# ChicyChen/LOCO-Edit

Hardware: AMD Instinct MI355X
Metric: edit-directions/sec (top-5 PMP-Jacobian SVD @256^2) + vT cos-sim vs ref (higher is better)
Workload: dtype bf16x3 (split-bf16 MFMA operands, fp32 accumulate + fp32 storage); 1 GPU; CelebA-HQ DDPM 256x256 top-5 local basis (l_eye-sized mask, L=2400), t=0.6T, 12 power iterations, one GPU; multi_gpu_form=single, probes_total=5, probes_per_gpu=5, kept=5, n_iter=12, mask_L=2400, weights=synthetic seed 0, streams=2

## Files before the change

include/loco_hip_diag.h:

```cpp
#ifndef LOCO_HIP_DIAG_H
#define LOCO_HIP_DIAG_H
#include "loco_hip.h"
#ifdef __cplusplus
extern "C" {
#endif

int  loco_bench_conv(loco_ctx* ctx, int32_t cin, int32_t cout, int32_t H, int32_t W, int32_t B, int32_t mode,
                     int32_t taps, int32_t tile, int32_t iters, float* ms_avg, void* stream);

typedef struct loco_conv_desc {
    int32_t struct_size;
    int32_t Cin, Cout, Hin, Win, B, taps;
    int32_t stride, upsample, zins, mode, cpg;
    int32_t transposed, accumulate, in_arena, pad;
    int32_t Cin2, cot_cpg;
    float   res_scale;
    int32_t st_cpg;
    const float *weight, *bias;
    const float *in, *bias2, *res;
    const float *prim, *sc, *sh, *mr, *gamma, *tst, *tc;
    const float *in2, *w2, *bias2nd;
    const float *cot_d, *cot_prim, *cot_sc, *cot_sh, *cot_mr, *cot_tc;
    float* out;
    const float *st_prim, *st_mr;
    float* st_out;
    int32_t pool2;
} loco_conv_desc;
int  loco_debug_conv(loco_ctx* ctx, const loco_conv_desc* desc, char* plan, int64_t cap, void* stream);

int64_t loco_debug_tensor(loco_ctx* ctx, const char* name, float* dst, int64_t cap, void* stream);

#ifdef __cplusplus
}
#endif
#endif
```

loco-edit_amd/csrc/engine.hip:

```cpp
#include <hip/hip_runtime.h>

#include <algorithm>
#include <array>
#include <cmath>
#include <cstdio>
#include <cstdlib>
#include <cstring>
#include <map>
#include <memory>
#include <thread>
#include <atomic>
#include <string>
#include <vector>

#include "../../include/loco_hip.h"
#ifdef LOCO_DIAG
#include "../../include/loco_hip_diag.h"
#endif
#include "kernels.h"
#include "program.h"
#ifdef LOCO_DIAG
#include "conv_plan_text.h"
#endif

// ... 49 lines not shown

struct Tens : TensPlan {
    float* keep = nullptr; size_t keep_floats = 0; int keep_ntile = 0;
};
struct NormP : NormPlan, NormW {
    bool ready = false;
};
struct Op : OpPlan, OpWeights {
    NormP n1, n2, nx;
    float *xK = nullptr, *xV = nullptr;
};

struct HostParam { std::vector<float> data; std::vector<int64_t> shape; bool loaded = false; };

}


struct loco_ctx {
    loco_unet_cfg cfg;
    std::string err;
    std::map<std::string, HostParam> params;
    bool finalized = false;

    std::shared_ptr<const Program> prog;
    std::shared_ptr<Weights> wts;
    std::vector<Tens> tens;
    std::vector<Op> ops;


    float *arenaP = nullptr, *arenaT = nullptr;
    float *statsP = nullptr, *statsT = nullptr;
    double* red = nullptr;
    bool fuse_cot = true;
    float *stpart = nullptr, *stpart2 = nullptr;
    size_t stpart_floats = 0;
    bool fuse_stats = true;
    bool fuse_xattn = true;
    bool deep1 = true;
    bool flash_attn = true;
    float* attn_delta = nullptr;
    float* partial = nullptr;
    size_t partial_floats = 0;
    const float* bench_out = nullptr; int64_t bench_out_count = 0;
#ifdef LOCO_DIAG
    std::string* plan_log = nullptr;
#endif
    float *tact = nullptr, *tproj = nullptr;
    float* eps_buf = nullptr;
    float* gx0 = nullptr;
    float* ge = nullptr;
    float* tmpA = nullptr;
    double *G = nullptr, *Q = nullptr, *W = nullptr, *gscratch = nullptr;
    float* alphas = nullptr;
    float* ctx_colbias = nullptr;
    bool has_ctx = false;
    float* cond_add = nullptr;
    float* ctx_norm = nullptr;
    bool has_cond = false;
    float* cond_in = nullptr;
    bool has_tcond = false;
    float2* sxcache = nullptr;
    int prec = 0;
    std::vector<float*> owned;
    size_t bytes = 0;

    bool primal_ok = false;
// ... 477 lines not shown
#endif
    if (rq && rq->kind != ST_NONE && rq->n) rq->n->ready = true;
    if (rq && rq->keep_ntile) *rq->keep_ntile = p.keep_ntile;
    const int HWo = a.Hout * a.Wout, Gn = c->cfg.gn_groups;
    const long SBs = c->prog->stats_per_sample;
    auto timed = [&](const char* name, double flops, const ConvArgs& y, auto&& launch) {
        loco_ctx::ProfRec r;
        if (c->prof_on) {
            r.name = name; r.flops = flops;
            r.cin = y.Cin; r.cout = y.Cout; r.h = y.Hout; r.b = y.B; r.ns = y.nsplit; r.mode = y.mode; r.taps = taps;
            r.e0 = c->next_event(); r.e1 = c->next_event();
            (void)hipEventRecord(r.e0, st);
        }
        launch();
        if (c->prof_on) { (void)hipEventRecord(r.e1, st); c->prof.push_back(r); }
    };
    for (int li = 0; li < p.nl; ++li) {
        const ConvLaunch& l = p.l[li];
        const ConvArgs& x = l.args;
        double flops = 2.0 * (x.Cin * taps + x.Cin2) * x.Cout * (double)x.Hout * x.Wout * x.B;
        if (x.zins) flops *= 0.25;
        if (x.poly == 2) flops *= 4.0;
        timed(c->prof_on ? conv_variant_name(x, taps, c->prec) : nullptr, flops, x, [&] {
            if (c->prec == 1) launch_conv_bf16x3(x, taps, st);
            else if (c->prec == 2) launch_conv_f16(x, taps, st);
            else launch_conv(x, taps, st);
        });
        if (x.nsplit > 1) {
            timed("conv_splitk_reduce", 0.0, x, [&] {
                if (l.stats != SR_SPLITK) { launch_conv_splitk_reduce(x, st); return; }
                const NormP& n = *rq->n;
                NS sp = nstats(c, c->statsP, n);
                NS so = nstats(c, rq->stats + (long)l.s0 * SBs, n);
                launch_conv_splitk_reduce_stats(x, rq->kind, Gn, eps_of(c, n), n.gamma, n.beta, so.mr, so.sc, so.sh, SBs, rq->ss_scale,
                                                rq->ss_shift, rq->prim, sp.sc, sp.sh, sp.mr, so.tst, so.tc, SBs, c->red, st);
            });
        }
        if (l.stats == SR_ALONE) stats_standalone(c, *rq, x.out, x.out_bs, x.B, HWo, l.s0, st);
        if (l.stats == SR_EPI) {
            const NormP& n = *rq->n;
            NS so = nstats(c, rq->stats + (long)l.s0 * SBs, n);
            if (rq->kind != ST_FWD) {
                NS sp = nstats(c, c->statsP, n);
                launch_gn_lin_fused_finalize(rq->kind, x.st_part, n.C, l.ntile, nullptr, 0, x.B, n.C, HWo, Gn, sp.mr, so.tst, so.tc,
                                             SBs, st);
            } else {
                launch_gn_fused_finalize(x.st_part, l.ntile, x.B, n.C, HWo, Gn, eps_of(c, n), n.gamma, n.beta, so.mr, so.sc, so.sh,
                                         SBs, rq->ss_scale, rq->ss_shift, st);
            }
        }
    }
    if (p.stats_all) stats_standalone(c, *rq, a.out, a.out_bs, a.B, HWo, 0, st);
    if (p.pool_after)
        launch_pool2x2_sum(a.pool_tmp, a.pool_tmp_bs, p.pool_out, p.pool_out_bs, p.pool_acc, a.B, a.Cout, a.Hout, a.Wout, st);
    return p.cot;
}

inline void setw(ConvArgs& a, const ConvP& p, bool dgrad) {
    a.w = dgrad ? p.wd : p.wf;
    a.wb = dgrad ? (const void*)p.wbd : (const void*)p.wbf;
    a.wh = dgrad ? (const void*)p.whd : (const void*)p.whf;
    const bool folded = p.wpb && p.poly_dgrad == dgrad;
    a.wpb = folded ? p.wpb : nullptr;
    a.wph = folded ? p.wph : nullptr;
    a.wqb = dgrad ? p.wqb : nullptr;
    a.wqh = dgrad ? p.wqh : nullptr;
}
// ... 904 lines not shown
    for (size_t i = 0; i < P.ops.size(); ++i) {
        const OpPlan& plan = P.ops[i];
        Op& v = c->ops[i];
        static_cast<OpPlan&>(v) = plan;
        static_cast<NormPlan&>(v.n1) = plan.n1; static_cast<NormPlan&>(v.n2) = plan.n2; static_cast<NormPlan&>(v.nx) = plan.nx;
        if (!plan.has_ctx_kv()) continue;
        const size_t kv = (size_t)P.tens[plan.in].C * P.ctx_Lp;
        if (dalloc(c, &v.xK, kv) || dalloc(c, &v.xV, kv)) return -1;
    }
    return 0;
}

int create_ctx(loco_ctx* c, const loco_unet_cfg* cfg, std::shared_ptr<const Program> prog) {
    c->cfg = *cfg;
    c->prog = std::move(prog);
    const size_t MB = (size_t)cfg->max_batch;
    {
        float *p0 = nullptr, *p1 = nullptr;
        if (dalloc(c, &p0, MB * c->prog->per_sample + 128) || dalloc(c, &p1, MB * c->prog->per_sample + 128)) return -1;
        c->arenaP = p0 + 64; c->arenaT = p1 + 64;
    }
    if (dalloc(c, &c->statsP, MB * c->prog->stats_per_sample) || dalloc(c, &c->statsT, MB * c->prog->stats_per_sample)) return -1;
    if (dalloc(c, &c->red, RED_BYTES) || dalloc(c, &c->red2, RED_BYTES)) return -1;
    if (alloc_state(c)) return -1;
    {
        c->stpart_floats = MB * (size_t)(c->prog->max_tensor / 64 + 1) * 2;
        if (dalloc(c, &c->stpart, c->stpart_floats) || dalloc(c, &c->stpart2, c->stpart_floats)) return -1;
        const char* e = getenv("LOCO_FUSE_STATS");
        c->fuse_stats = !(e && atoi(e) == 0);
        e = getenv("LOCO_FUSE_LIN");
        c->fuse_lin = !(e && atoi(e) == 0);
        e = getenv("LOCO_FUSE_COT");
        c->fuse_cot = !(e && atoi(e) == 0) && cfg->act == ACT_SILU;
        e = getenv("LOCO_DEEP1");
        c->deep1 = !(e && atoi(e) == 0);
        e = getenv("LOCO_FUSE_XATTN");
        c->fuse_xattn = !(e && atoi(e) == 0);
        const char* fa = getenv("LOCO_FLASH_ATTN");
        c->flash_attn = !(fa && atoi(fa) == 0);
        if (dalloc(c, &c->attn_delta, MB * (size_t)c->prog->attn_dmax)) return -1;
    }
    c->partial_floats = (size_t)64 << 20;
    if (dalloc(c, &c->partial, c->partial_floats)) return -1;
    if (dalloc(c, &c->xin_buf, MB * c->prog->n_in) || dalloc(c, &c->t_dev, 4)) return -1;
    if (dalloc(c, &c->eps_buf, MB * c->prog->n_out) || dalloc(c, &c->gx0, MB * c->prog->n_in) || dalloc(c, &c->ge, MB * c->prog->n_out))
        return -1;
    if (dalloc(c, &c->tmpA, (size_t)64 * c->prog->n_in)) return -1;
    if (dalloc(c, &c->G, 64 * 64) || dalloc(c, &c->Q, 64 * 64) || dalloc(c, &c->W, SOLVER_W_GATE + 1)) return -1;
    {
        size_t nblk = ((size_t)c->prog->n_in + 255) / 256;
        if (dalloc(c, &c->gscratch, nblk * 64 * 64 + 4096)) return -1;
    }
    if (dalloc(c, &c->alphas, 256) || dalloc(c, &c->cond_add, (size_t)cfg->ch * 4)) return -1;
    if (dalloc(c, &c->cond_in, (size_t)cfg->ch)) return -1;
    {
        float2* sx0 = nullptr;
        if (dalloc(c, &sx0, (size_t)c->prog->sx_total + 64)) return -1;
        c->sxcache = sx0 + 32;
    }
    {
        const char* e = getenv("LOCO_PRECISION");
        c->prec = (e && std::string(e) == "f32") ? 0 : (e && std::string(e) == "f16") ? 2 : 1;
    }
    if (dalloc(c, &c->mask2, (size_t)c->prog->n_out)) return -1;
    if (dalloc(c, &c->mask, (size_t)c->prog->n_out) || dalloc(c, &c->mask_idx, (size_t)c->prog->n_out) ||
        dalloc(c, &c->mask_L_dev, 4)) return -1;
// ... 695 lines not shown
    const int taps = d->taps, k = taps == 9 ? 3 : 1, B = d->B;
    if ((taps != 9 && taps != 1) || d->Cin < 1 || d->Cout < 1 || d->Hin < 1 || d->Win < 1 || B < 1 || (d->stride != 1 && d->stride != 2) ||
        d->mode < CM_NONE || d->mode > CM_GN_GELU || (d->upsample && d->zins) || (d->stride == 2 && (d->upsample || d->zins)) ||
        !d->weight || !d->in || !d->out) { c->err = "debug_conv: bad descriptor"; return -2; }
    if (d->stride == 2 && ((d->Hin | d->Win) & 1)) { c->err = "debug_conv: stride 2 needs an even map"; return -2; }
    const bool lin = d->mode == CM_TAN_SILU || d->mode == CM_COT_SILU;
    if (d->mode != CM_NONE && (!d->sc || !d->sh)) { c->err = "debug_conv: the prologue modes need sc / sh"; return -2; }
    if (lin && (!d->prim || !d->mr || !d->gamma || !d->tst || !d->tc || d->cpg < 1 || d->Cin % d->cpg)) {
        c->err = "debug_conv: modes 3 / 4 need prim, mr, gamma, tst, tc and cpg"; return -2;
    }
    if (d->Cin2 > 0 && (!d->in2 || !d->w2)) { c->err = "debug_conv: the second operator needs in2 and w2"; return -2; }
    if (d->Cin2 > 0 && (d->res || d->accumulate || taps != 9)) {
        c->err = "debug_conv: the second operator goes with a 3x3 conv without res / accumulate"; return -2;
    }
    if (d->cot_d && (!d->cot_prim || !d->cot_sc || !d->cot_sh || !d->cot_mr || !d->cot_tc || d->cot_cpg < 1 || d->Cout % d->cot_cpg)) {
        c->err = "debug_conv: the norm-cotangent term needs cot_prim, cot_sc, cot_sh, cot_mr, cot_tc and cot_cpg"; return -2;
    }
    if (d->pool2 && (taps != 9 || d->stride != 1 || d->upsample || d->zins || d->mode != CM_NONE || d->Cin2 > 0 || d->res || d->cot_d ||
                     ((d->Hin | d->Win) & 1))) { c->err = "debug_conv: pool2 goes with a raw 3x3 stride-1 conv of an even map"; return -2; }
    const int Hout = (d->stride == 2 || d->pool2) ? d->Hin / 2 : (d->upsample || d->zins) ? 2 * d->Hin : d->Hin;
    const int Wout = (d->stride == 2 || d->pool2) ? d->Win / 2 : (d->upsample || d->zins) ? 2 * d->Win : d->Win;
    {
        auto pow2 = [](int v) { return v >= 8 && (v & (v - 1)) == 0; };
        auto walks = [&](int h, int w) { return (pow2(h) && pow2(w)) || (w % 32 == 0 && h % 8 == 0 && ((long)h * w) % 256 == 0); };
        if (!walks(Hout, Wout) || (d->pool2 && !walks(d->Hin, d->Win))) {
            c->err = "debug_conv: output map outside the tile geometry of the conv kernels"; return -2;
        }
    }
    const long in_e = (long)d->Cin * d->Hin * d->Win, out_e = (long)d->Cout * Hout * Wout, in2_e = (long)d->Cin2 * Hout * Wout;
    if ((in_e | out_e | in2_e) & 3) { c->err = "debug_conv: planes must be whole 16-byte units"; return -2; }
    auto up64 = [](long v) { return (v + 63) & ~63L; };
    const long offT_in2 = d->in_arena ? up64(in_e * B) : 0, offT_cot = offT_in2 + up64(in2_e * B);
    const long needT = offT_cot + (d->cot_d ? out_e * B : 0);
    const long sx_cot = lin ? up64(in_e) : 0, need_sx = sx_cot + (d->cot_d ? out_e : 0);
    if (needT > (long)c->cfg.max_batch * c->prog->per_sample || (lin && in_e > (long)c->cfg.max_batch * c->prog->per_sample) ||
        need_sx > c->prog->sx_total) { c->err = "debug_conv: shape exceeds the arenas"; return -2; }
    const int G = lin ? d->Cin / d->cpg : 0;
    const long tbs = up64(2L * G) + up64(2L * d->Cin);
    const bool st_req = d->st_prim != nullptr;
    if (st_req && (!d->st_mr || !d->st_out || d->st_cpg < 1 || d->Cout % d->st_cpg || d->cot_d || d->Cin2 > 0)) {
        c->err = "debug_conv: the statistics request needs st_prim, st_mr, st_out and st_cpg (no second operator, no cot_d)"; return -2;
    }
    const long keep_n = st_req ? up64((long)B * d->Cout * ((long)Hout * Wout / 64 + 1) * 2) : 0;
    const long small_n = (lin ? (long)B * tbs : 0) + (d->cot_d ? (long)B * up64(2L * d->Cout) : 0) + 64 + keep_n + (st_req ? up64(2L * d->Cout) : 0);
    const size_t owned0 = c->owned.size();
    const size_t bytes0 = c->bytes;
    auto release = [&]() {
        (void)hipStreamSynchronize(st);
        while (c->owned.size() > owned0) { (void)hipFree(c->owned.back()); c->owned.pop_back(); }
        c->bytes = bytes0;
    };
    auto host_param = [&](const float* p, std::vector<int64_t> shape) {
        HostParam h; h.shape = shape; h.loaded = true;
        size_t n = 1; for (int64_t s : shape) n *= (size_t)s;
        if (p) h.data.assign(p, p + n); else h.data.assign(n, 0.f);
        return h;
    };
    const int m_out = d->transposed ? d->Cin : d->Cout, m_in = d->transposed ? d->Cout : d->Cin;
    HostParam w = host_param(d->weight, {m_out, m_in, k, k}), wb0 = host_param(nullptr, {m_out});
    HostParam w2 = host_param(d->Cin2 > 0 ? d->w2 : nullptr, {d->Cout, d->Cin2 > 0 ? d->Cin2 : 1, 1, 1}), wb2 = host_param(nullptr, {d->Cout});
    ConvP cp, cp2;
    float *bias_d = nullptr, *bias2nd_d = nullptr, *small = nullptr;
    const int poly_kind = taps != 9 ? -1 : (d->upsample || d->pool2) ? POLY_UP : d->zins ? ((d->pad >= 0 ? d->pad : 2) == 1 ? POLY_ZINS_PAD1 : POLY_ZINS_PAD2) : -1;
    int rc = make_conv(c, {&w}, {&wb0}, &cp, -1, poly_kind, d->transposed != 0 && !d->pool2);
    float* pool_tmp = nullptr;
    if (!rc && d->pool2) rc = dalloc(c, &pool_tmp, (size_t)B * d->Cout * d->Hin * d->Win);
    if (!rc && d->Cin2 > 0) rc = make_conv(c, {&w2}, {&wb2}, &cp2);
// ... 31 lines not shown
        a.sx = c->sxcache;
    }
    ConvArgs n2; conv_defaults(n2);
    if (d->Cin2 > 0) {
        float* in2 = c->arenaT + offT_in2;
        if (he == hipSuccess) he = copy(in2, d->in2, in2_e * B);
        n2.in = in2; n2.in_bs = in2_e; n2.Cin = d->Cin2; n2.Hin = Hout; n2.Win = Wout;
        setw(n2, cp2, false); n2.bias = bias2nd_d; n2.pad = 0;
        n2.out = d->out; n2.out_bs = out_e; n2.Cout = d->Cout; n2.Hout = Hout; n2.Wout = Wout; n2.B = B;
        a.res = d->out; a.res_bs = out_e;
    }
    if (d->cot_d) {
        float* cd = c->arenaT + offT_cot;
        float* ctc = small + (lin ? (long)B * tbs : 0);
        const long cbs = up64(2L * d->Cout);
        if (he == hipSuccess) he = copy(cd, d->cot_d, out_e * B);
        for (int b = 0; b < B; ++b)
            hipLaunchKernelGGL(diag_scale_tc, dim3((unsigned)((d->Cout + 255) / 256)), dim3(256), 0, st, d->cot_tc + (long)b * 2 * d->Cout,
                               d->cot_mr, d->Cout, d->cot_cpg, (long)d->Cout, 1, ctc + b * cbs);
        launch_gn_cache(d->cot_prim, d->Cout, Hout * Wout, d->cot_cpg, d->cot_sc, d->cot_sh, d->cot_mr, c->sxcache + sx_cot, st, ACT_SILU);
        a.cot_d = cd; a.cot_d_bs = out_e; a.cot_sx = c->sxcache + sx_cot; a.cot_tc = ctc; a.cot_tc_bs = cbs;
    }
    if (he != hipSuccess) { c->err = std::string("debug_conv: ") + hipGetErrorString(he); release(); return -1; }
    std::string text;
    const int act0 = c->cfg.act;
    if (d->mode == CM_GN_GELU) c->cfg.act = ACT_GELU;
    c->plan_log = &text;
    StatReq srq;
    int kept_ntile = 0;
    float* const keep_buf = small + (small_n - keep_n - (st_req ? up64(2L * d->Cout) : 0));
    if (st_req) {
        srq.kind = ST_TAN; srq.prim = d->st_prim; srq.keep = keep_buf; srq.keep_floats = (size_t)keep_n; srq.keep_ntile = &kept_ntile;
    }
    const bool rode = run_conv(c, a, taps, st, st_req ? &srq : nullptr, d->Cin2 > 0 ? &n2 : nullptr);
    c->plan_log = nullptr;
    c->cfg.act = act0;
    if (st_req) {
        const int G2 = d->Cout / d->st_cpg;
        float* const zero = keep_buf + keep_n;
        (void)hipMemsetAsync(zero, 0, (size_t)up64(2L * d->Cout) * sizeof(float), st);
        (void)hipMemsetAsync(d->st_out, 0xff, (size_t)B * G2 * 2 * sizeof(float), st);
        if (kept_ntile > 0)
            launch_gn_lin_fused_finalize(ST_TAN, keep_buf, d->Cout, kept_ntile, nullptr, 0, B, d->Cout, Hout * Wout, G2, d->st_mr, d->st_out,
                                         nullptr, 2L * G2, st);
        launch_gn_tstats(d->out, out_e, d->st_prim, 0, B, d->Cout, Hout * Wout, G2, zero, zero + d->Cout, d->st_mr, 0, 0, 0,
                         d->st_out + (long)B * G2 * 2, nullptr, 2L * G2, c->red, st, ACT_SILU);
    }
    he = hipGetLastError();
    release();
    if (he == hipSuccess) he = hipGetLastError();
    if (he != hipSuccess) { c->err = std::string("debug_conv: ") + hipGetErrorString(he); return -1; }
    if (plan && cap > 0) {
        if ((int64_t)text.size() + 1 > cap) { c->err = "debug_conv: plan buffer too small"; return -4; }
        std::memcpy(plan, text.c_str(), text.size() + 1);
    }
    if (d->cot_d && !rode) { c->err = "debug_conv: norm-cotangent term declined"; return 1; }
    return 0;
}

#endif

int loco_set_streams(loco_ctx* c, int32_t n) {
    if (!c || (n != 1 && n != 2)) return -2;
    c->n_streams = n;
    return 0;
}

int loco_set_chip_share(loco_ctx* c, int32_t n) {
    if (!c || n < 1 || n > 8) return -2;
// ... 84 lines not shown
```

loco-edit_amd/csrc/misc.hip:

```cpp
#include "kernels.h"

namespace loco {

typedef float f32x4_t __attribute__((ext_vector_type(4)));

__device__ __forceinline__ double wave_sum(double v) {
#pragma unroll
    for (int o = 32; o > 0; o >>= 1) v += __shfl_down(v, o, 64);
    return v;
}
__device__ __forceinline__ float wave_sumf(float v) {
#pragma unroll
    for (int o = 32; o > 0; o >>= 1) v += __shfl_down(v, o, 64);
    return v;
}
__device__ __forceinline__ float wave_maxf(float v) {
#pragma unroll
    for (int o = 32; o > 0; o >>= 1) v = fmaxf(v, __shfl_down(v, o, 64));
    return v;
}
__device__ __forceinline__ double block_sum(double v, double* sm) {
    v = wave_sum(v);
    __syncthreads();
    if ((threadIdx.x & 63) == 0) sm[threadIdx.x >> 6] = v;
    __syncthreads();
    double r = 0.0;
    for (int i = 0; i < (int)(blockDim.x >> 6); ++i) r += sm[i];
    return r;
}

__global__ __launch_bounds__(256) void gn_partial_kernel(const float* x, long bs, long len, double* scratch) {
    __shared__ double sm[4];
    const int s = blockIdx.x, nsplit = gridDim.x, g = blockIdx.y, b = blockIdx.z, G = gridDim.y;
    const float* p = x + (long)b * bs + (long)g * len;
    long per = ((len / 4 + nsplit - 1) / nsplit) * 4;
    long beg = (long)s * per, end = beg + per < len ? beg + per : len;
    if (beg > end) beg = end;
    const long n4 = (end - beg) / 4;
    const float4* p4 = reinterpret_cast<const float4*>(p + beg);
    double sum = 0.0;
    for (long i = threadIdx.x; i < n4; i += 256) {
        float4 v = p4[i];
        sum += (double)((v.x + v.y) + (v.z + v.w));
    }
    for (long i = beg + n4 * 4 + threadIdx.x; i < end; i += 256) sum += (double)p[i];
    double tot = block_sum(sum, sm);
    const double cnt = (double)(end - beg);
    const float mean = cnt > 0 ? (float)(tot / cnt) : 0.f;
    double m2 = 0.0;
    for (long i = threadIdx.x; i < n4; i += 256) {
        float4 v = p4[i];
        float a0 = v.x - mean, a1 = v.y - mean, a2 = v.z - mean, a3 = v.w - mean;
        m2 += (double)((a0 * a0 + a1 * a1) + (a2 * a2 + a3 * a3));
    }
    for (long i = beg + n4 * 4 + threadIdx.x; i < end; i += 256) {
        float a0 = p[i] - mean;
        m2 += (double)(a0 * a0);
    }
    double M2 = block_sum(m2, sm);
    if (threadIdx.x == 0) {
        double* o = scratch + (((long)b * G + g) * nsplit + s) * 3;
// ... 286 lines not shown
        float* o = tst + (long)b * tbs + 2 * g;
        o[0] = m1;
        o[1] = m2;
    }
    if (tc) {
        const float f = kind == ST_TAN ? 1.0f : rstd;
        for (int k = threadIdx.x; k < cpg; k += 256) {
            float* t = tc + (long)b * tbs + 2 * ((long)g * cpg + k);
            t[0] = f * m1;
            t[1] = f * m2;
        }
    }
}
void launch_gn_lin_fused_finalize(int kind, const float* partA, int C1, int ntA, const float* partB, int ntB, int B, int C, int HW,
                                  int G, const float* mr, float* tst, float* tc, long tst_bs, hipStream_t st) {
    hipLaunchKernelGGL(gn_lin_fused_finalize_kernel, dim3(G, B), dim3(256), 0, st, kind, partA, C1, ntA, partB, ntB, C, G,
                       1.0 / ((double)(C / G) * HW), mr, tst, tc, tst_bs);
}
void launch_gn_fused_finalize_cat(const float* partA, int C1, int ntA, const float* partB, int ntB, int B, int C, int HW, int G,
                                  float eps, const float* gamma, const float* beta, float* mr, float* sc, float* sh,
                                  long stats_bs, hipStream_t st) {
    hipLaunchKernelGGL(gn_fused_finalize_cat_kernel, dim3(G, B), dim3(64), 0, st, partA, C1, ntA, partB, ntB, C, G, HW, eps,
                       gamma, beta, mr, sc, sh, stats_bs);
}

void launch_gn_fused_finalize(const float* part, int ntile, int B, int C, int HW, int G, float eps, const float* gamma,
                              const float* beta, float* mr, float* sc, float* sh, long stats_bs, const float* ss_scale,
                              const float* ss_shift, hipStream_t st) {
    const double inv_n = 1.0 / ((double)(C / G) * HW);
    hipLaunchKernelGGL(gn_fused_finalize_kernel, dim3(G, B), dim3(64), 0, st, part, ntile, C, G, inv_n, eps, gamma, beta, mr,
                       sc, sh, stats_bs, ss_scale, ss_shift);
}

template <int KIND>
__global__ __launch_bounds__(1024) void splitk_reduce_stats_kernel(ConvArgs a, int G, float eps, const float* gamma,
                                                                  const float* beta, float* mr, float* sc, float* sh, long sbs,
                                                                  const float* ss_scale, const float* ss_shift,
                                                                  const float* prim, const float* sc_p, const float* sh_p,
                                                                  const float* mr_p, float* tst, float* tc, long tbs,
                                                                  double* scratch) {
    __shared__ double sm[16];
    const int s = blockIdx.x, nsl = gridDim.x, g = blockIdx.y, b = blockIdx.z;
    const int HW = a.Hout * a.Wout, cpg = a.Cout / G;
    const long step = (long)blockDim.x * 4;
    const long len = (long)cpg * HW, per_b = (long)a.Cout * HW, total = per_b * a.B;
    const long base = (long)g * len;
    long per = ((len / 4 + nsl - 1) / nsl) * 4;
    long beg = (long)s * per, end = beg + per < len ? beg + per : len;
    if (beg > end) beg = end;
    float mean_p = 0.f, rstd_p = 1.f;
    if (KIND != ST_FWD) { mean_p = mr_p[2 * g]; rstd_p = mr_p[2 * g + 1]; }
    double t1 = 0.0, t2 = 0.0;
    for (long i = beg + threadIdx.x * 4; i < end; i += step) {
        const long e = base + i;
        const int c = (int)(e / HW);
        f32x4_t v = {0.f, 0.f, 0.f, 0.f};
        const float* pp = a.partial + (long)b * per_b + e;
        int k = 0;
        for (; k + 4 <= a.nsplit; k += 4) {
            const f32x4_t p0 = *reinterpret_cast<const f32x4_t*>(pp + (long)k * total);
            const f32x4_t p1 = *reinterpret_cast<const f32x4_t*>(pp + (long)(k + 1) * total);
            const f32x4_t p2 = *reinterpret_cast<const f32x4_t*>(pp + (long)(k + 2) * total);
            const f32x4_t p3 = *reinterpret_cast<const f32x4_t*>(pp + (long)(k + 3) * total);
            v += (p0 + p1) + (p2 + p3);
        }
        for (; k < a.nsplit; ++k) v += *reinterpret_cast<const f32x4_t*>(pp + (long)k * total);
        float add = 0.f;
        if (a.bias) add += a.bias[c];
        if (a.bias2) add += a.bias2[(long)b * a.bias2_bs + c];
        v += add;
        if (a.res) v += a.res_scale * *reinterpret_cast<const f32x4_t*>(a.res + (long)b * a.res_bs + e);
        float* o = a.out + (long)b * a.out_bs + e;
        if (a.accumulate) v += *reinterpret_cast<const f32x4_t*>(o);
        *reinterpret_cast<f32x4_t*>(o) = v;
        float a1, a2;
        if (KIND == ST_FWD) {
            a1 = (v[0] + v[1]) + (v[2] + v[3]);
            a2 = 0.f;
        } else {
            const f32x4_t xv = *reinterpret_cast<const f32x4_t*>(prim + e);
            const float scc = sc_p[c], shc = sh_p[c];
            a1 = 0.f; a2 = 0.f;
#pragma unroll
            for (int j = 0; j < 4; ++j) {
                const float xh = (xv[j] - mean_p) * rstd_p;
                float z = v[j];
                if (KIND == ST_COT) z *= (scc / rstd_p) * act_der(fmaf(scc, xv[j], shc), a.act);
                a1 += z;
                a2 += xh * z;
            }
        }
        t1 += (double)a1;
        t2 += (double)a2;
    }
    t1 = block_sum(t1, sm);
    if (KIND == ST_FWD) {
        const double n = (double)(end - beg);
        const float mu = n > 0 ? (float)(t1 / n) : 0.f;
        double m2 = 0.0;
        for (long i = beg + threadIdx.x * 4; i < end; i += step) {
            const f32x4_t v = *reinterpret_cast<const f32x4_t*>(a.out + (long)b * a.out_bs + base + i);
            const float d0 = v[0] - mu, d1 = v[1] - mu, d2 = v[2] - mu, d3 = v[3] - mu;
            m2 += (double)((d0 * d0 + d1 * d1) + (d2 * d2 + d3 * d3));
        }
        const double dm = (n > 0 ? t1 / n : 0.0) - (double)mu;
        t2 = block_sum(m2, sm) - n * dm * dm;
    } else {
        t2 = block_sum(t2, sm);
    }
    if (nsl > 1) {
        if (threadIdx.x == 0) {
            if (KIND == ST_FWD) {
                double* o = scratch + (((long)b * G + g) * nsl + s) * 3;
                const double n = (double)(end - beg), mu = n > 0 ? t1 / n : 0.0;
                o[0] = n; o[1] = mu; o[2] = t2;
            } else {
                double* o = scratch + (((long)b * G + g) * nsl + s) * 2;
                o[0] = t1; o[1] = t2;
            }
        }
        return;
    }
    const double inv_n = 1.0 / (double)len;
    if (KIND == ST_FWD) {
        const double mean = t1 * inv_n;
        double var = t2 * inv_n;
        if (var < 0.0) var = 0.0;
        const float meanf = (float)mean, rstd = (float)(1.0 / sqrt(var + (double)eps));
        if (threadIdx.x == 0) {
            mr[(long)b * sbs + g * 2] = meanf;
            mr[(long)b * sbs + g * 2 + 1] = rstd;
        }
        if (threadIdx.x < cpg) {
            const int c = g * cpg + threadIdx.x;
            const float gm = gamma[c];
            float aa = gm * rstd, oo = beta[c] - meanf * rstd * gm;
            if (ss_scale) {
                const float f = 1.0f + ss_scale[c];
                aa *= f;
                oo = oo * f + ss_shift[c];
            }
            sc[(long)b * sbs + c] = aa;
            sh[(long)b * sbs + c] = oo;
        }
    } else {
        const float m1 = (float)(t1 * inv_n), m2 = (float)(t2 * inv_n);
        if (threadIdx.x == 0) {
            tst[(long)b * tbs + 2 * g] = m1;
            tst[(long)b * tbs + 2 * g + 1] = m2;
        }
        if (tc && threadIdx.x < cpg) {
            const float f = KIND == ST_TAN ? 1.0f : rstd_p;
            float* t = tc + (long)b * tbs + 2 * ((long)g * cpg + threadIdx.x);
            t[0] = f * m1;
            t[1] = f * m2;
        }
    }
}

void launch_conv_splitk_reduce_stats(const ConvArgs& a, int kind, int G, float eps, const float* gamma, const float* beta,
                                     float* mr, float* sc, float* sh, long stats_bs, const float* ss_scale,
                                     const float* ss_shift, const float* prim, const float* sc_prim, const float* sh_prim,
                                     const float* mr_prim, float* tst, float* tc, long tst_bs, double* scratch,
                                     hipStream_t st) {
    const int HW = a.Hout * a.Wout, cpg = a.Cout / G;
    const long len = (long)cpg * HW;
    const int ns = gn_nsplit(len, a.B * G);
    dim3 grid(ns, G, a.B);
    long pieces = (len / ns + 3) / 4;
    int nthr = (int)((pieces + 63) / 64) * 64;
    if (nthr < 64) nthr = 64;
    if (nthr > 1024) nthr = 1024;
    if (nthr < cpg) nthr = ((cpg + 63) / 64) * 64;
#define RS(K) hipLaunchKernelGGL(splitk_reduce_stats_kernel<K>, grid, dim3(nthr), 0, st, a, G, eps, gamma, beta, mr, sc, sh, \
                                 stats_bs, ss_scale, ss_shift, prim, sc_prim, sh_prim, mr_prim, tst, tc, tst_bs, scratch)
    if (kind == ST_FWD) RS(ST_FWD); else if (kind == ST_TAN) RS(ST_TAN); else RS(ST_COT);
#undef RS
    if (ns == 1) return;
    if (kind == ST_FWD) {
        hipLaunchKernelGGL(gn_finalize_kernel, dim3((G + 63) / 64, a.B), dim3(64), 0, st, scratch, ns, G, a.Cout, eps, gamma,
                           beta, mr, sc, sh, stats_bs, ss_scale, ss_shift);
    } else {
        const long BG = (long)a.B * G;
        hipLaunchKernelGGL(gn_tstats_finalize, dim3((unsigned)((BG + 255) / 256)), dim3(256), 0, st, scratch, ns, BG, G,
                           1.0 / (double)len, tst, tc, tst_bs, cpg, mr_prim, 0L, kind == ST_TAN ? 0 : 1);
    }
}

template <int KIND>
__global__ __launch_bounds__(256) void gn_apply_kernel(const float* d, long d_bs, const float* x, long x_bs,
                                                       const float* base, long base_bs, float* out, long out_bs,
                                                       int accumulate, int C, int HW, int cpg, const float* sc,
                                                       const float* sh, const float* mr, long pbs_c, long pbs_g,
                                                       const float* tst, long tbs, int act, float base_scale) {
    const int b = blockIdx.y;
    const long per = (long)C * HW;
    for (long i = ((long)blockIdx.x * 256 + threadIdx.x) * 4; i < per; i += (long)gridDim.x * 1024) {
        int c = (int)(i / HW);
        int g = c / cpg;
        float scc = sc[(long)b * pbs_c + c], shc = sh[(long)b * pbs_c + c];
        float4 xv = *reinterpret_cast<const float4*>(x + (long)b * x_bs + i);
        float xx[4] = {xv.x, xv.y, xv.z, xv.w};
        float r[4];
        if (KIND == 0) {
#pragma unroll
            for (int j = 0; j < 4; ++j) r[j] = fmaf(scc, xx[j], shc);
        } else if (KIND == 4) {
#pragma unroll
            for (int j = 0; j < 4; ++j) r[j] = act_fwd(fmaf(scc, xx[j], shc), act);
// ... 439 lines not shown
```

loco-edit_amd/hip.py:

```python
from __future__ import annotations

import ctypes as C
import os
from typing import Dict, Optional

import numpy as np
import torch

from .config import UNetConfig

_LIB_PATH = os.environ.get("LOCO_HIP_LIB") or os.path.join(os.path.dirname(os.path.abspath(__file__)), "libloco_hip.so")
_lib = None

DIAG_SYMBOLS = ["loco_bench_conv", "loco_debug_conv", "loco_debug_tensor"]

SYMBOLS = [
    "loco_version", "loco_device_count", "loco_create", "loco_fork", "loco_destroy", "loco_last_error",
    "loco_load_param", "loco_params_missing", "loco_unet_forward", "loco_ddim_step", "loco_sched_step",
    "loco_pmp_primal", "loco_pmp_set_second_mask", "loco_pmp_jvp", "loco_pmp_vjp", "loco_orthonormalize", "loco_qr_rows",
    "loco_convergence", "loco_convergence_rows", "loco_null_project", "loco_edit_axpy", "loco_mask_gather", "loco_mask_count",
    "loco_unet_flops", "loco_workspace_bytes", "loco_clock_stamp", "loco_set_side_stream", "loco_timer_start", "loco_timer_stop",
    "loco_profile_enable", "loco_profile_report", "loco_set_precision", "loco_get_precision", "loco_set_streams", "loco_set_chip_share",
    "loco_set_cond", "loco_set_context", "loco_lincomb", "loco_masked_axpby", "loco_latent_sample",
    "loco_text_create", "loco_text_load_param", "loco_text_params_missing", "loco_text_encode", "loco_text_last_error",
    "loco_text_destroy", "loco_t5_create", "loco_text_encode_masked",
    "loco_diffedit_mask", "loco_cfg_masked_step", "loco_set_time_cond", "loco_lcm_step",
    "loco_sam_create", "loco_sam_load_param", "loco_sam_params_missing", "loco_sam_encode", "loco_sam_profile",
    "loco_sam_profile_read", "loco_sam_last_error", "loco_sam_destroy",
    "loco_samdec_create", "loco_samdec_load_param", "loco_samdec_params_missing", "loco_samdec_set_image", "loco_samdec_predict",
    "loco_samdec_score", "loco_samdec_binarize", "loco_samdec_last_error", "loco_samdec_destroy",
    "loco_clipvis_create", "loco_clipvis_load_param", "loco_clipvis_params_missing", "loco_clipvis_preprocess",
    "loco_clipvis_encode", "loco_clipvis_last_error", "loco_clipvis_destroy",
    "loco_quality_create", "loco_quality_load_param", "loco_quality_params_missing", "loco_quality_lpips", "loco_quality_ssim",
    "loco_quality_masked_mse", "loco_quality_last_error", "loco_quality_destroy",
]

DIFFEDIT_RULES = {"reference": 0, "intended": 1}


class LocoCfg(C.Structure):
    _fields_ = [
        ("struct_size", C.c_int32), ("resolution", C.c_int32), ("in_channels", C.c_int32), ("out_ch", C.c_int32), ("ch", C.c_int32),
        ("num_levels", C.c_int32), ("ch_mult", C.c_int32 * 8), ("num_res_blocks", C.c_int32),
        ("num_attn_res", C.c_int32), ("attn_resolutions", C.c_int32 * 8), ("gn_groups", C.c_int32),
        ("gn_eps", C.c_float), ("max_batch", C.c_int32),
        ("arch", C.c_int32), ("num_head_channels", C.c_int32), ("learn_sigma", C.c_int32),
        ("context_dim", C.c_int32), ("context_len", C.c_int32),
        ("scale_shift_norm", C.c_int32), ("resblock_updown", C.c_int32), ("num_heads", C.c_int32),
        ("transformer_depth", C.c_int32),
        ("act", C.c_int32), ("res_scale", C.c_float), ("added_kv", C.c_int32),
        ("time_cond_proj_dim", C.c_int32),
    ]


class LocoConvDesc(C.Structure):
    _PTRS = ("weight", "bias", "in", "bias2", "res", "prim", "sc", "sh", "mr", "gamma", "tst", "tc", "in2", "w2", "bias2nd",
             "cot_d", "cot_prim", "cot_sc", "cot_sh", "cot_mr", "cot_tc", "out", "st_prim", "st_mr", "st_out")
    _HOST = ("weight", "bias", "w2", "bias2nd")
    _fields_ = ([("struct_size", C.c_int32)] +
                [(k, C.c_int32) for k in ("Cin", "Cout", "Hin", "Win", "B", "taps", "stride", "upsample", "zins", "mode", "cpg",
                                          "transposed", "accumulate", "in_arena", "pad", "Cin2", "cot_cpg")] +
                [("res_scale", C.c_float), ("st_cpg", C.c_int32)] + [(k, C.c_void_p) for k in _PTRS] + [("pool2", C.c_int32)])


class LocoTextCfg(C.Structure):
    _fields_ = [("vocab", C.c_int32), ("width", C.c_int32), ("layers", C.c_int32), ("heads", C.c_int32), ("ffn", C.c_int32),
                ("positions", C.c_int32), ("act", C.c_int32), ("ln_eps", C.c_float)]


class LocoT5Cfg(C.Structure):
    _fields_ = [("vocab", C.c_int32), ("d_model", C.c_int32), ("d_kv", C.c_int32), ("heads", C.c_int32), ("d_ff", C.c_int32),
                ("layers", C.c_int32), ("positions", C.c_int32), ("buckets", C.c_int32), ("max_distance", C.c_int32),
                ("act", C.c_int32), ("ln_eps", C.c_float)]


SAM_MAX_GLOBAL = 16


class LocoSamCfg(C.Structure):
    _fields_ = [("image_size", C.c_int32), ("patch_size", C.c_int32), ("width", C.c_int32), ("depth", C.c_int32),
                ("heads", C.c_int32), ("mlp_dim", C.c_int32), ("window_size", C.c_int32), ("num_global", C.c_int32),
                ("global_attn", C.c_int32 * SAM_MAX_GLOBAL), ("out_channels", C.c_int32), ("ln_eps", C.c_float)]


class LocoSamDecCfg(C.Structure):
    _fields_ = [("grid", C.c_int32), ("image_size", C.c_int32), ("hidden", C.c_int32), ("layers", C.c_int32), ("heads", C.c_int32),
                ("mlp_dim", C.c_int32), ("attention_downsample_rate", C.c_int32), ("num_multimask_outputs", C.c_int32),
                ("iou_head_depth", C.c_int32), ("iou_head_hidden_dim", C.c_int32), ("layer_norm_eps", C.c_float),
                ("hidden_act", C.c_int32), ("max_prompts", C.c_int32)]


class LocoClipVisCfg(C.Structure):
    _fields_ = [("image_size", C.c_int32), ("patch_size", C.c_int32), ("width", C.c_int32), ("layers", C.c_int32),
                ("heads", C.c_int32), ("mlp_dim", C.c_int32), ("projection_dim", C.c_int32), ("act", C.c_int32),
                ("ln_eps", C.c_float), ("image_mean", C.c_float * 3), ("image_std", C.c_float * 3)]
# ... 553 lines not shown
            side = BranchStreams._pick(1, self.device)
            if not side:
                self.set_streams(1)
                return 1
            self.set_side_stream(side[0])
        self.set_streams(n)
        return n

    def get_precision(self) -> str:
        m = self.lib.loco_get_precision(self._ctx)
        return {v: k for k, v in self.PRECISIONS.items()}[m]

    def _need_diag(self, sym):
        if not hasattr(self.lib, sym):
            raise RuntimeError(f"{sym} is a diagnostic of include/loco_hip_diag.h: build `make -C loco-edit_amd/csrc diag` "
                               "and set LOCO_HIP_LIB=<repo>/loco-edit_amd/libloco_hip_diag.so")

    def bench_conv(self, cin, cout, H, W, B, mode, taps=9, tile=-1, iters=20) -> float:
        self._need_diag("loco_bench_conv")
        ms = C.c_float()
        self._check(self.lib.loco_bench_conv(self._ctx, cin, cout, H, W, B, mode, taps, tile, iters, C.byref(ms),
                                             _stream()), "loco_bench_conv")
        return float(ms.value)

    def debug_conv(self, out: torch.Tensor, **desc):
        self._need_diag("loco_debug_conv")
        d = LocoConvDesc()
        d.struct_size = C.sizeof(LocoConvDesc)
        d.stride, d.in_arena, d.pad, d.res_scale = 1, 1, -1, 1.0
        keep = []
        _chk_dev(out)
        d.out = out.data_ptr()
        for k, v in desc.items():
            if k not in LocoConvDesc._PTRS:
                if not hasattr(d, k) or k == "struct_size":
                    raise TypeError(f"debug_conv: no descriptor field {k!r}")
                setattr(d, k, v)
            elif v is not None:
                if k in LocoConvDesc._HOST:
                    v = v.detach().to("cpu", torch.float32).contiguous()
                else:
                    _chk_dev(v)
                keep.append(v)
                setattr(d, k, v.data_ptr())
        buf = C.create_string_buffer(1 << 12)
        rc = self.lib.loco_debug_conv(self._ctx, C.byref(d), buf, len(buf), _stream())
        if rc not in (0, 1):
            self._check(rc, "loco_debug_conv")
        plan = []
        for line in buf.value.decode().splitlines():
            rec = dict(f.split("=", 1) for f in line.split(" "))
            plan.append({k: (v if k == "kernel" else int(v)) for k, v in rec.items()})
        return plan, rc == 0

    def profile_enable(self, on):
        self._check(self.lib.loco_profile_enable(self._ctx, int(on)), "loco_profile_enable")

    def profile_report(self):
        buf = C.create_string_buffer(1 << 18)
        self._check(self.lib.loco_profile_report(self._ctx, buf, len(buf)), "loco_profile_report")
        out = {}
        for line in buf.value.decode().splitlines():
            name, n, ms, fl = line.rsplit(" ", 3)
            out[name] = dict(launches=int(float(n)), ms=float(ms), flops=float(fl))
        return out

    def debug_tensor(self, name: str, numel: int) -> torch.Tensor:
# ... 333 lines not shown
```

Measured before the change: 20.35 edit-directions/s.

## Overhaul split-K reduce-stats kernel: cached cotangent records, slab-templated loads, register reuse

Reworks the split-K reduce plus group-norm statistics kernel. It templates the number of partial slabs so all loads are issued up front. The cotangent path reads precomputed scale/x-hat records from the sx cache instead of recomputing the activation derivative. Forward mode keeps the first few reduced vectors in registers for the variance pass, and the two block sums are merged into one. It also replaces 64-bit division with shifts or 32-bit division and adds diagnostic hooks for the norm-stats path, at the cost of more template instances and extra register pressure.

```diff
diff --git a/include/loco_hip_diag.h b/include/loco_hip_diag.h
--- a/include/loco_hip_diag.h
+++ b/include/loco_hip_diag.h
@@ -25,6 +25,9 @@
     const float *st_prim, *st_mr;
     float* st_out;
     int32_t pool2;
+    int32_t sn_kind, sn_records;
+    const float *sn_gamma, *sn_beta, *sn_prim, *sn_sc, *sn_sh, *sn_mr;
+    float* sn_out;
 } loco_conv_desc;
 int  loco_debug_conv(loco_ctx* ctx, const loco_conv_desc* desc, char* plan, int64_t cap, void* stream);
 
diff --git a/loco-edit_amd/csrc/engine.hip b/loco-edit_amd/csrc/engine.hip
--- a/loco-edit_amd/csrc/engine.hip
+++ b/loco-edit_amd/csrc/engine.hip
@@ -105,6 +105,7 @@
     float *statsP = nullptr, *statsT = nullptr;
     double* red = nullptr;
     bool fuse_cot = true;
+    bool splitk_cot_rec = true;
     float *stpart = nullptr, *stpart2 = nullptr;
     size_t stpart_floats = 0;
     bool fuse_stats = true;
@@ -648,7 +649,10 @@
                 const NormP& n = *rq->n;
                 NS sp = nstats(c, c->statsP, n);
                 NS so = nstats(c, rq->stats + (long)l.s0 * SBs, n);
-                launch_conv_splitk_reduce_stats(x, rq->kind, Gn, eps_of(c, n), n.gamma, n.beta, so.mr, so.sc, so.sh, SBs, rq->ss_scale,
+                ConvArgs y = x;
+                y.st_sx = (rq->kind == ST_COT && c->splitk_cot_rec && c->prec >= 1 && n.sx_off >= 0 && c->sxcache) ? c->sxcache + n.sx_off
+                                                                                                                     : nullptr;
+                launch_conv_splitk_reduce_stats(y, rq->kind, Gn, eps_of(c, n), n.gamma, n.beta, so.mr, so.sc, so.sh, SBs, rq->ss_scale,
                                                 rq->ss_shift, rq->prim, sp.sc, sp.sh, sp.mr, so.tst, so.tc, SBs, c->red, st);
             });
         }
@@ -1619,6 +1623,8 @@
         c->fuse_lin = !(e && atoi(e) == 0);
         e = getenv("LOCO_FUSE_COT");
         c->fuse_cot = !(e && atoi(e) == 0) && cfg->act == ACT_SILU;
+        e = getenv("LOCO_SPLITK_COT_REC");
+        c->splitk_cot_rec = !(e && atoi(e) == 0);
         e = getenv("LOCO_DEEP1");
         c->deep1 = !(e && atoi(e) == 0);
         e = getenv("LOCO_FUSE_XATTN");
@@ -2380,7 +2386,16 @@
     auto up64 = [](long v) { return (v + 63) & ~63L; };
     const long offT_in2 = d->in_arena ? up64(in_e * B) : 0, offT_cot = offT_in2 + up64(in2_e * B);
     const long needT = offT_cot + (d->cot_d ? out_e * B : 0);
-    const long sx_cot = lin ? up64(in_e) : 0, need_sx = sx_cot + (d->cot_d ? out_e : 0);
+    const bool sn_req = d->sn_kind != ST_NONE;
+    const int Gn = c->cfg.gn_groups;
+    if (sn_req && (d->sn_kind < ST_FWD || d->sn_kind > ST_COT || d->Cout % Gn || !d->sn_out || d->st_prim || d->cot_d || d->Cin2 > 0 ||
+                   d->pool2 || (d->sn_kind == ST_FWD ? (!d->sn_gamma || !d->sn_beta) : (!d->sn_prim || !d->sn_sc || !d->sn_sh || !d->sn_mr)))) {
+        c->err = "debug_conv: the norm statistics request needs sn_out, Cout a multiple of the groups, sn_gamma / sn_beta (forward) or "
+                 "sn_prim, sn_sc, sn_sh, sn_mr (tangent, cotangent); no second operator, cot_d, st_prim or pool2";
+        return -2;
+    }
+    const bool sn_rec = sn_req && d->sn_kind == ST_COT && d->sn_records;
+    const long sx_cot = lin ? up64(in_e) : 0, need_sx = sx_cot + ((d->cot_d || sn_rec) ? out_e : 0);
     if (needT > (long)c->cfg.max_batch * c->prog->per_sample || (lin && in_e > (long)c->cfg.max_batch * c->prog->per_sample) ||
         need_sx > c->prog->sx_total) { c->err = "debug_conv: shape exceeds the arenas"; return -2; }
     const int G = lin ? d->Cin / d->cpg : 0;
@@ -2478,9 +2493,33 @@
     if (st_req) {
         srq.kind = ST_TAN; srq.prim = d->st_prim; srq.keep = keep_buf; srq.keep_floats = (size_t)keep_n; srq.keep_ntile = &kept_ntile;
     }
-    const bool rode = run_conv(c, a, taps, st, st_req ? &srq : nullptr, d->Cin2 > 0 ? &n2 : nullptr);
+    NormP dn;
+    float* const statsP0 = c->statsP;
+    const long sn_slot = 4L * d->Cout + 4L * Gn, SBs = c->prog->stats_per_sample;
+    float *sn_primal = nullptr, *sn_stats = nullptr;
+    if (sn_req) {
+        const size_t stats_n = (size_t)((B - 1) * SBs + sn_slot);
+        if (dalloc(c, &sn_primal, (size_t)sn_slot) || dalloc(c, &sn_stats, stats_n)) { c->plan_log = nullptr; c->cfg.act = act0; release(); return -1; }
+        dn.C = d->Cout; dn.soff = 0;
+        dn.gamma = const_cast<float*>(d->sn_gamma); dn.beta = const_cast<float*>(d->sn_beta);
+        (void)hipMemsetAsync(sn_stats, 0xff, stats_n * sizeof(float), st);
+        if (d->sn_kind != ST_FWD) {
+            NS sp = nstats(c, sn_primal, dn);
+            (void)copy(sp.sc, d->sn_sc, d->Cout); (void)copy(sp.sh, d->sn_sh, d->Cout); (void)copy(sp.mr, d->sn_mr, 2L * Gn);
+            if (sn_rec) {
+                launch_gn_cache(d->sn_prim, d->Cout, Hout * Wout, d->Cout / Gn, d->sn_sc, d->sn_sh, d->sn_mr, c->sxcache + sx_cot, st, c->cfg.act);
+                dn.sx_off = sx_cot;
+            }
+        }
+        srq.kind = d->sn_kind; srq.n = &dn; srq.stats = sn_stats; srq.prim = d->sn_prim;
+        c->statsP = sn_primal;
+    }
+    const bool rode = run_conv(c, a, taps, st, (st_req || sn_req) ? &srq : nullptr, d->Cin2 > 0 ? &n2 : nullptr);
+    c->statsP = statsP0;
     c->plan_log = nullptr;
     c->cfg.act = act0;
+    if (sn_req)
+        for (int b = 0; b < B; ++b) (void)copy(d->sn_out + (long)b * sn_slot, sn_stats + (long)b * SBs, sn_slot);
     if (st_req) {
         const int G2 = d->Cout / d->st_cpg;
         float* const zero = keep_buf + keep_n;
diff --git a/loco-edit_amd/csrc/misc.hip b/loco-edit_amd/csrc/misc.hip
--- a/loco-edit_amd/csrc/misc.hip
+++ b/loco-edit_amd/csrc/misc.hip
@@ -27,6 +27,17 @@
     double r = 0.0;
     for (int i = 0; i < (int)(blockDim.x >> 6); ++i) r += sm[i];
     return r;
+}
+__device__ __forceinline__ void block_sum2(double& a, double& b, double* sm) {
+    a = wave_sum(a);
+    b = wave_sum(b);
+    __syncthreads();
+    if ((threadIdx.x & 63) == 0) { sm[threadIdx.x >> 6] = a; sm[16 + (threadIdx.x >> 6)] = b; }
+    __syncthreads();
+    double ra = 0.0, rb = 0.0;
+    for (int i = 0; i < (int)(blockDim.x >> 6); ++i) { ra += sm[i]; rb += sm[16 + i]; }
+    a = ra;
+    b = rb;
 }
 
 __global__ __launch_bounds__(256) void gn_partial_kernel(const float* x, long bs, long len, double* scratch) {
@@ -379,14 +390,45 @@
                        sc, sh, stats_bs, ss_scale, ss_shift);
 }
 
-template <int KIND>
+constexpr int SPLITK_KEEP = 4;
+template <int NSLAB>
+__device__ __forceinline__ void splitk_load(const float* pp, long total, int k0, int nsplit, f32x4_t (&p)[NSLAB]) {
+#pragma unroll
+    for (int j = 0; j < NSLAB; ++j) {
+        const int k = k0 + j < nsplit ? k0 + j : nsplit - 1;
+        p[j] = *reinterpret_cast<const f32x4_t*>(pp + (long)k * total);
+    }
+}
+template <int NSLAB>
+__device__ __forceinline__ f32x4_t splitk_add(f32x4_t v, const f32x4_t (&p)[NSLAB], int k0, int nsplit) {
+    static_assert(NSLAB % 4 == 0, "whole groups of four");
+#pragma unroll
+    for (int j = 0; j < NSLAB; j += 4) {
+        if (k0 + j + 4 <= nsplit) v += (p[j] + p[j + 1]) + (p[j + 2] + p[j + 3]);
+        else {
+#pragma unroll
+            for (int r = 0; r < 4; ++r)
+                if (k0 + j + r < nsplit) v += p[j + r];
+        }
+    }
+    return v;
+}
+static int splitk_chunk(int nsplit) { return nsplit <= 4 ? 4 : nsplit <= 8 ? 8 : nsplit <= 12 ? 12 : 16; }
+static int splitk_pow2_shift(long v) {
+    if (v <= 0 || (v & (v - 1))) return -1;
+    int s = 0;
+    while ((1L << s) < v) ++s;
+    return s;
+}
+
+template <int KIND, int NSLAB>
 __global__ __launch_bounds__(1024) void splitk_reduce_stats_kernel(ConvArgs a, int G, float eps, const float* gamma,
                                                                   const float* beta, float* mr, float* sc, float* sh, long sbs,
                                                                   const float* ss_scale, const float* ss_shift,
                                                                   const float* prim, const float* sc_p, const float* sh_p,
-                                                                  const float* mr_p, float* tst, float* tc, long tbs,
-                                                                  double* scratch) {
-    __shared__ double sm[16];
+                                                                  const float* mr_p, const float2* sx_p, int hw_shift, float* tst,
+                                                                  float* tc, long tbs, double* scratch) {
+    __shared__ double sm[32];
     const int s = blockIdx.x, nsl = gridDim.x, g = blockIdx.y, b = blockIdx.z;
     const int HW = a.Hout * a.Wout, cpg = a.Cout / G;
     const long step = (long)blockDim.x * 4;
@@ -395,65 +437,122 @@
     long per = ((len / 4 + nsl - 1) / nsl) * 4;
     long beg = (long)s * per, end = beg + per < len ? beg + per : len;
     if (beg > end) beg = end;
+    const bool rec = KIND == ST_COT && sx_p != nullptr;
+    const bool idx32 = per_b <= 0x7fffffffL;
     float mean_p = 0.f, rstd_p = 1.f;
     if (KIND != ST_FWD) { mean_p = mr_p[2 * g]; rstd_p = mr_p[2 * g + 1]; }
-    double t1 = 0.0, t2 = 0.0;
-    for (long i = beg + threadIdx.x * 4; i < end; i += step) {
+    auto piece = [&](long i, float& a1, float& a2) -> f32x4_t {
         const long e = base + i;
-        const int c = (int)(e / HW);
+        const float* pp = a.partial + (long)b * per_b + e;
+        f32x4_t p[NSLAB];
+        splitk_load<NSLAB>(pp, total, 0, a.nsplit, p);
+        const int c = hw_shift >= 0 ? (int)(e >> hw_shift) : idx32 ? (int)((unsigned)e / (unsigned)HW) : (int)(e / HW);
+        float* o = a.out + (long)b * a.out_bs + e;
+        const float add = *(a.bias ? a.bias + c : pp);
+        const float add2 = *(a.bias2 ? a.bias2 + (long)b * a.bias2_bs + c : pp);
+        const f32x4_t rv = *reinterpret_cast<const f32x4_t*>(a.res ? a.res + (long)b * a.res_bs + e : pp);
+        const f32x4_t ov = *reinterpret_cast<const f32x4_t*>(a.accumulate ? o : pp);
+        float scc = 0.f, shc = 0.f;
+        f32x4_t x0 = {0.f, 0.f, 0.f, 0.f}, x1 = {0.f, 0.f, 0.f, 0.f};
+        if (KIND == ST_TAN) x0 = *reinterpret_cast<const f32x4_t*>(prim + e);
+        if (KIND == ST_COT) {
+            const float* q = rec ? reinterpret_cast<const float*>(sx_p + e) : prim + e;
+            x0 = *reinterpret_cast<const f32x4_t*>(q);
+            x1 = *reinterpret_cast<const f32x4_t*>(rec ? q + 4 : q);
+            scc = sc_p[c];
+            shc = sh_p[c];
+        }
         f32x4_t v = {0.f, 0.f, 0.f, 0.f};
-        const float* pp = a.partial + (long)b * per_b + e;
-        int k = 0;
-        for (; k + 4 <= a.nsplit; k += 4) {
-            const f32x4_t p0 = *reinterpret_cast<const f32x4_t*>(pp + (long)k * total);
-            const f32x4_t p1 = *reinterpret_cast<const f32x4_t*>(pp + (long)(k + 1) * total);
-            const f32x4_t p2 = *reinterpret_cast<const f32x4_t*>(pp + (long)(k + 2) * total);
-            const f32x4_t p3 = *reinterpret_cast<const f32x4_t*>(pp + (long)(k + 3) * total);
-            v += (p0 + p1) + (p2 + p3);
-        }
-        for (; k < a.nsplit; ++k) v += *reinterpret_cast<const f32x4_t*>(pp + (long)k * total);
-        float add = 0.f;
-        if (a.bias) add += a.bias[c];
-        if (a.bias2) add += a.bias2[(long)b * a.bias2_bs + c];
-        v += add;
-        if (a.res) v += a.res_scale * *reinterpret_cast<const f32x4_t*>(a.res + (long)b * a.res_bs + e);
-        float* o = a.out + (long)b * a.out_bs + e;
-        if (a.accumulate) v += *reinterpret_cast<const f32x4_t*>(o);
+        v = splitk_add<NSLAB>(v, p, 0, a.nsplit);
+        if (NSLAB == 16) {
+            for (int k0 = NSLAB; k0 < a.nsplit; k0 += NSLAB) {
+                splitk_load<NSLAB>(pp, total, k0, a.nsplit, p);
+                v = splitk_add<NSLAB>(v, p, k0, a.nsplit);
+            }
+        }
+        float bsum = 0.f;
+        if (a.bias) bsum += add;
+        if (a.bias2) bsum += add2;
+        v += bsum;
+        if (a.res) v += a.res_scale * rv;
+        if (a.accumulate) v += ov;
         *reinterpret_cast<f32x4_t*>(o) = v;
-        float a1, a2;
         if (KIND == ST_FWD) {
             a1 = (v[0] + v[1]) + (v[2] + v[3]);
             a2 = 0.f;
+        } else if (rec) {
+            const float S[4] = {x0[0], x0[2], x1[0], x1[2]}, xr[4] = {x0[1], x0[3], x1[1], x1[3]};
+            a1 = 0.f; a2 = 0.f;
+#pragma unroll
+            for (int j = 0; j < 4; ++j) {
+                const float z = __fmul_rn(v[j], S[j]);
+                a1 = __fadd_rn(a1, z);
+                a2 = fmaf(xr[j], z, a2);
+            }
         } else {
-            const f32x4_t xv = *reinterpret_cast<const f32x4_t*>(prim + e);
-            const float scc = sc_p[c], shc = sh_p[c];
             a1 = 0.f; a2 = 0.f;
 #pragma unroll
             for (int j = 0; j < 4; ++j) {
-                const float xh = (xv[j] - mean_p) * rstd_p;
-                float z = v[j];
-                if (KIND == ST_COT) z *= (scc / rstd_p) * act_der(fmaf(scc, xv[j], shc), a.act);
-                a1 += z;
-                a2 += xh * z;
+                const float xh = (x0[j] - mean_p) * rstd_p;
+                if (KIND == ST_COT) {
+                    const float T = (scc / rstd_p) * act_der(fmaf(scc, x0[j], shc), a.act);
+                    a1 = fmaf(v[j], T, a1);
+                    a2 = fmaf(xh, __fmul_rn(v[j], T), a2);
+                } else {
+                    a1 = __fadd_rn(a1, v[j]);
+                    a2 = __fadd_rn(a2, __fmul_rn(xh, v[j]));
+                }
             }
         }
+        return v;
+    };
+    double t1 = 0.0, t2 = 0.0;
+    const long i0 = beg + threadIdx.x * 4;
+    f32x4_t keep[SPLITK_KEEP];
+    if (KIND == ST_FWD) {
+#pragma unroll
+        for (int q = 0; q < SPLITK_KEEP; ++q) {
+            keep[q] = f32x4_t{0.f, 0.f, 0.f, 0.f};
+            if (i0 + q * step < end) {
+                float a1, a2;
+                keep[q] = piece(i0 + q * step, a1, a2);
+                t1 += (double)a1;
+            }
+        }
+    }
+    for (long i = KIND == ST_FWD ? i0 + SPLITK_KEEP * step : i0; i < end; i += step) {
+        float a1, a2;
+        piece(i, a1, a2);
         t1 += (double)a1;
         t2 += (double)a2;
     }
-    t1 = block_sum(t1, sm);
     if (KIND == ST_FWD) {
+        t1 = block_sum(t1, sm);
         const double n = (double)(end - beg);
         const float mu = n > 0 ? (float)(t1 / n) : 0.f;
         double m2 = 0.0;
-        for (long i = beg + threadIdx.x * 4; i < end; i += step) {
+#pragma unroll
+        for (int q = 0; q < SPLITK_KEEP; ++q) {
+            if (i0 + q * step < end) {
+                const f32x4_t v = keep[q];
+                const float d0 = v[0] - mu, d1 = v[1] - mu, d2 = v[2] - mu, d3 = v[3] - mu;
+                m2 += (double)__fadd_rn(fmaf(d0, d0, __fmul_rn(d1, d1)), fmaf(d2, d2, __fmul_rn(d3, d3)));
+            }
+        }
+        for (long i = i0 + SPLITK_KEEP * step; i < end; i += step) {
             const f32x4_t v = *reinterpret_cast<const f32x4_t*>(a.out + (long)b * a.out_bs + base + i);
             const float d0 = v[0] - mu, d1 = v[1] - mu, d2 = v[2] - mu, d3 = v[3] - mu;
-            m2 += (double)((d0 * d0 + d1 * d1) + (d2 * d2 + d3 * d3));
+            m2 += (double)__fadd_rn(fmaf(d0, d0, __fmul_rn(d1, d1)), fmaf(d2, d2, __fmul_rn(d3, d3)));
         }
         const double dm = (n > 0 ? t1 / n : 0.0) - (double)mu;
         t2 = block_sum(m2, sm) - n * dm * dm;
     } else {
-        t2 = block_sum(t2, sm);
+        block_sum2(t1, t2, sm);
+        if (rec) {
+            const double ir = 1.0 / (double)rstd_p;
+            t1 *= ir;
+            t2 *= ir;
+        }
     }
     if (nsl > 1) {
         if (threadIdx.x == 0) {
@@ -510,7 +609,9 @@
                                      const float* ss_shift, const float* prim, const float* sc_prim, const float* sh_prim,
                                      const float* mr_prim, float* tst, float* tc, long tst_bs, double* scratch,
                                      hipStream_t st) {
+    const float2* sx = kind == ST_COT ? a.st_sx : nullptr;
     const int HW = a.Hout * a.Wout, cpg = a.Cout / G;
+    const int shift = splitk_pow2_shift(HW);
     const long len = (long)cpg * HW;
     const int ns = gn_nsplit(len, a.B * G);
     dim3 grid(ns, G, a.B);
@@ -519,9 +620,12 @@
     if (nthr < 64) nthr = 64;
     if (nthr > 1024) nthr = 1024;
     if (nthr < cpg) nthr = ((cpg + 63) / 64) * 64;
-#define RS(K) hipLaunchKernelGGL(splitk_reduce_stats_kernel<K>, grid, dim3(nthr), 0, st, a, G, eps, gamma, beta, mr, sc, sh, \
-                                 stats_bs, ss_scale, ss_shift, prim, sc_prim, sh_prim, mr_prim, tst, tc, tst_bs, scratch)
-    if (kind == ST_FWD) RS(ST_FWD); else if (kind == ST_TAN) RS(ST_TAN); else RS(ST_COT);
+#define RS(K, N) hipLaunchKernelGGL((splitk_reduce_stats_kernel<K, N>), grid, dim3(nthr), 0, st, a, G, eps, gamma, beta, mr, sc, sh, \
+                                    stats_bs, ss_scale, ss_shift, prim, sc_prim, sh_prim, mr_prim, sx, shift, tst, tc, tst_bs, scratch)
+#define RSN(K) do { switch (splitk_chunk(a.nsplit)) { case 4: RS(K, 4); break; case 8: RS(K, 8); break; case 12: RS(K, 12); break; \
+                                                      default: RS(K, 16); break; } } while (0)
+    if (kind == ST_FWD) RSN(ST_FWD); else if (kind == ST_TAN) RSN(ST_TAN); else RSN(ST_COT);
+#undef RSN
 #undef RS
     if (ns == 1) return;
     if (kind == ST_FWD) {
diff --git a/loco-edit_amd/hip.py b/loco-edit_amd/hip.py
--- a/loco-edit_amd/hip.py
+++ b/loco-edit_amd/hip.py
@@ -56,11 +56,13 @@
 class LocoConvDesc(C.Structure):
     _PTRS = ("weight", "bias", "in", "bias2", "res", "prim", "sc", "sh", "mr", "gamma", "tst", "tc", "in2", "w2", "bias2nd",
              "cot_d", "cot_prim", "cot_sc", "cot_sh", "cot_mr", "cot_tc", "out", "st_prim", "st_mr", "st_out")
+    _SN_PTRS = ("sn_gamma", "sn_beta", "sn_prim", "sn_sc", "sn_sh", "sn_mr", "sn_out")
     _HOST = ("weight", "bias", "w2", "bias2nd")
     _fields_ = ([("struct_size", C.c_int32)] +
                 [(k, C.c_int32) for k in ("Cin", "Cout", "Hin", "Win", "B", "taps", "stride", "upsample", "zins", "mode", "cpg",
                                           "transposed", "accumulate", "in_arena", "pad", "Cin2", "cot_cpg")] +
-                [("res_scale", C.c_float), ("st_cpg", C.c_int32)] + [(k, C.c_void_p) for k in _PTRS] + [("pool2", C.c_int32)])
+                [("res_scale", C.c_float), ("st_cpg", C.c_int32)] + [(k, C.c_void_p) for k in _PTRS] +
+                [(k, C.c_int32) for k in ("pool2", "sn_kind", "sn_records")] + [(k, C.c_void_p) for k in _SN_PTRS])
 
 
 class LocoTextCfg(C.Structure):
@@ -680,7 +682,7 @@
         _chk_dev(out)
         d.out = out.data_ptr()
         for k, v in desc.items():
-            if k not in LocoConvDesc._PTRS:
+            if k not in LocoConvDesc._PTRS + LocoConvDesc._SN_PTRS:
                 if not hasattr(d, k) or k == "struct_size":
                     raise TypeError(f"debug_conv: no descriptor field {k!r}")
                 setattr(d, k, v)
```

Result: no change. 20.39 edit-directions/s, median of 6 (+0.2%).
